# Golbstein/Keras-segmentation-deeplab-v3.1

Hardware: AMD Instinct MI355X
Metric: images/sec fwd+bwd, 512x512 MobileNetV2 OS=16, 21 classes (higher is better)
Workload: dtype f32; 1 GPU; Deeplabv3(backbone='mobilenetv2', input_shape=(512,512,3), classes=21, OS=16) head=deeplab: fwd + sparse-xent loss + bwd + Adam, BN batch mode, dropout 0.1; global_batch=128, per_gpu_batch=128, parallelism=dp1, hipgraph=True, matrix_math=f32, dist_strict=False, backward_fork=False

## Files before the change

### keras-segmentation-deeplab-v3.1_amd/csrc/dwconv.hip

```cpp
#include "common.h"

#pragma clang fp contract(on)
#include <type_traits>
#include <stdlib.h>

namespace {

__device__ __forceinline__ f32x4 ld4_su(const float *base, unsigned byte_off) {
  return ld4(reinterpret_cast<const float *>(reinterpret_cast<const char *>(base) + byte_off));
}
__device__ __forceinline__ void st4_nt_su(float *base, unsigned byte_off, f32x4 v) {
  st4_nt(reinterpret_cast<float *>(reinterpret_cast<char *>(base) + byte_off), v);
}

struct DwGeom {
  int N, H, W, C, stride, rate, pad_t, pad_l, Ho, Wo;
  int prows;
};

struct DwMarch {
  int H, W, C, r, nchunk, TK, nxseg, nphase, ppb, nslab, ny, N;
  int prows;
  int fast;
};

struct DwChan {
  f32x4 wv[9], s, t;
  f32x4 kA, kB, kC, mu, is;
};
__device__ __forceinline__ DwChan dw_chan(int c, int C, const float *w, const float *sc, const float *sh,
                                          const float *cA = nullptr, const float *cB = nullptr, const float *cC = nullptr,
                                          bool stats = false, const float *xmean = nullptr, const float *xinvstd = nullptr) {
  DwChan cn;
  const int c4 = min(c, C - 4);
#pragma unroll
  for (int i = 0; i < 9; i++) cn.wv[i] = ld4(w + (size_t)i * C + c4);
  cn.s = splat4(1.f); cn.t = splat4(0.f);
  cn.kA = splat4(1.f); cn.kB = splat4(0.f); cn.kC = splat4(0.f); cn.mu = splat4(0.f); cn.is = splat4(0.f);
  if (sc) { cn.s = ld4(sc + c4); cn.t = ld4(sh + c4); }
  if (cA) { cn.kA = ld4(cA + c4); cn.kB = ld4(cB + c4); cn.kC = ld4(cC + c4); }
  if (stats) { cn.mu = ld4(xmean + c4); cn.is = ld4(xinvstd + c4); }
  return cn;
}

__device__ __forceinline__ f32x4 dw_dy(const DwChan &cn, f32x4 gv, f32x4 yv) { return cn.kA * gv + cn.kB * yv + cn.kC; }
__device__ __forceinline__ const float *dw_yr(const float *cA, const float *yraw, const float *g) { return cA ? yraw : g; }

template <int NV>
__device__ __forceinline__ void reduce_px(float (&v)[NV], float *lds ) {
  const int tid = threadIdx.x;
  const int wave = tid >> 6, cq = tid & 7;
#pragma unroll
  for (int i = 0; i < NV; i++) {
    float s = v[i];
    s += __shfl_xor(s, 8, 64);
    s += __shfl_xor(s, 16, 64);
    s += __shfl_xor(s, 32, 64);
    v[i] = s;
  }
  __syncthreads();
  if ((tid & 63) < 8) {
#pragma unroll
    for (int i = 0; i < NV; i++) lds[(wave * 8 + cq) * NV + i] = v[i];
  }
  __syncthreads();
  if (tid < 8) {
#pragma unroll
    for (int i = 0; i < NV; i++)
      v[i] = ((lds[(0 * 8 + cq) * NV + i] + lds[(1 * 8 + cq) * NV + i]) + lds[(2 * 8 + cq) * NV + i]) +
             lds[(3 * 8 + cq) * NV + i];
  }
}

__device__ __forceinline__ void write_stat_partial(float *part, int p, int C, int c, f32x4 s1, f32x4 s2) {
  float *d = part + ((size_t)p * C + c) * 2;
  d[0] = s1.x; d[1] = s2.x; d[2] = s1.y; d[3] = s2.y;
  d[4] = s1.z; d[5] = s2.z; d[6] = s1.w; d[7] = s2.w;
}

__device__ __forceinline__ void pad_stat_partial(float *part, int p, int written, int rows, int C, int c) {
  for (int q = p + written; q < rows; q += written) write_stat_partial(part, q, C, c, splat4(0.f), splat4(0.f));
}
__device__ __forceinline__ void pad_w_partial(float *wpart, int p, int written, int rows, int C, int c) {
  for (int q = p + written; q < rows; q += written)
#pragma unroll
    for (int i = 0; i < 9; i++) st4(wpart + ((size_t)q * 9 + i) * C + c, splat4(0.f));
}

__device__ __forceinline__ void dw_store_stats(float *part, int p, int written, int rows, int C, int c, f32x4 s1, f32x4 s2,
                                               float *red ) {
  if (!part) return;
  float v[8] = {s1.x, s1.y, s1.z, s1.w, s2.x, s2.y, s2.z, s2.w};
  reduce_px<8>(v, red);
  if (threadIdx.x < 8 && c < C) {
    f32x4 r1 = {v[0], v[1], v[2], v[3]}, r2 = {v[4], v[5], v[6], v[7]};
    write_stat_partial(part, p, C, c, r1, r2);
    pad_stat_partial(part, p, written, rows, C, c);
  }
}
__device__ __forceinline__ void dw_store_wgrad(float *wpart, int p, int written, int rows, int C, int c, const f32x4 (&dwv)[9],
                                               float *red ) {
  float v[36];
#pragma unroll
  for (int i = 0; i < 9; i++) {
    v[i * 4 + 0] = dwv[i].x; v[i * 4 + 1] = dwv[i].y; v[i * 4 + 2] = dwv[i].z; v[i * 4 + 3] = dwv[i].w;
  }
  reduce_px<36>(v, red);
  if (threadIdx.x < 8 && c < C) {
#pragma unroll
    for (int i = 0; i < 9; i++) {
      f32x4 o = {v[i * 4], v[i * 4 + 1], v[i * 4 + 2], v[i * 4 + 3]};
      st4(wpart + ((size_t)p * 9 + i) * C + c, o);
    }
    pad_w_partial(wpart, p, written, rows, C, c);
  }
}

struct DwTile { int xs, slab, pc, n; };
__device__ __forceinline__ bool dw_tile(const DwMarch &M, DwTile &t) {
  const int L = blockIdx.x, chunk = gridDim.x >> 3;
  int v = (L & 7) * chunk + (L >> 3);
  if (v >= M.nxseg * M.nslab * M.ny * M.N) return false;
  t.xs = v % M.nxseg; v /= M.nxseg;
  t.slab = v % M.nslab; v /= M.nslab;
  t.pc = v % M.ny;
  t.n = v / M.ny;
  t.xs = __builtin_amdgcn_readfirstlane(t.xs);
  t.slab = __builtin_amdgcn_readfirstlane(t.slab);
  t.pc = __builtin_amdgcn_readfirstlane(t.pc);
  t.n = __builtin_amdgcn_readfirstlane(t.n);
  return true;
}
__device__ __forceinline__ int dw_tile_row(const DwMarch &M, const DwTile &t) { return (t.n * M.ny + t.pc) * M.nxseg + t.xs; }

struct DwPhase {
  int a, Ka, k0, k1, Kc;
  bool bot_halo;
  int ks, ke;
};
__device__ __forceinline__ bool dw_phase(const DwMarch &M, int pc, int pi, DwPhase &ph) {
  const int a = __builtin_amdgcn_readfirstlane((M.ppb > 1) ? pc * M.ppb + pi : pc / M.nchunk);
  const int ch = __builtin_amdgcn_readfirstlane((M.ppb > 1) ? 0 : pc % M.nchunk);
  const int Ka = __builtin_amdgcn_readfirstlane((a < M.H) ? (M.H - a + M.r - 1) / M.r : 0);
  const int k0 = ch * M.TK;
  const int k1 = min(k0 + M.TK, Ka);
  const int Kc = max(Ka - 1, 0);
  const bool bot_halo = k1 < Ka;
  const int ks = (k0 > 0) ? k0 - 1 : k0, ke = bot_halo ? k1 : k1 - 1;
  ph = DwPhase{a, Ka, k0, k1, Kc, bot_halo, ks, ke};
  return a < M.nphase;
}

template <int R, class Group>
__device__ __forceinline__ void dw_walk(const DwPhase &ph, bool fast_ok, int fast_last, Group &group) {
  int kg = ph.ks;
  group(kg, std::false_type{});
  kg += R;
  if (fast_ok) {
    __builtin_amdgcn_s_waitcnt(0x0F70);
    for (; kg + R - 1 <= fast_last; kg += R) group(kg, std::true_type{});
  }
  for (; kg <= ph.ke; kg += R) group(kg, std::false_type{});
}

__global__ __launch_bounds__(256, 3) void dw_march_fwd(const float *__restrict__ x, const float *__restrict__ sc,
                                                    const float *__restrict__ sh, int act,
                                                    const float *__restrict__ w, float *__restrict__ y, DwMarch M,
                                                    float *__restrict__ part) {
  __shared__ float red[4 * 8 * 8];
  const int tid = threadIdx.x, cq = tid & 7, pl = tid >> 3;
  DwTile tile;
  if (!dw_tile(M, tile)) return;
  const int H = M.H, W = M.W, C = M.C, r = M.r;
  const int xs = tile.xs, slab = tile.slab, n = tile.n;
  const int c = slab * 32 + cq * 4;
  const int xx = xs * 32 + pl;
  const bool active = (c < C) && (xx < W);

  const DwChan cn = dw_chan(c, C, w, sc, sh);
  f32x4 s1 = splat4(0.f), s2 = splat4(0.f);
  for (int pi = 0; pi < M.ppb; ++pi) {
    DwPhase ph;
    if (!dw_phase(M, tile.pc, pi, ph)) break;
    const int a = ph.a;
    const bool xl_ok = (xx - r >= 0), xr_ok = (xx + r < W);
    const int cc = min(c, C - 4), xc = min(xx, W - 1), xlc = min(max(xx - r, 0), W - 1), xrc = min(xx + r, W - 1);
    const float *xn = x + (size_t)n * H * W * C;
    float *yn = y + (size_t)n * H * W * C;
    const unsigned om = 4u * (unsigned)(xc * C + cc), ol = 4u * (unsigned)(xlc * C + cc), orr = 4u * (unsigned)(xrc * C + cc);
    const unsigned oo = 4u * (unsigned)(xx * C + c);

    auto ldrow = [&](int k, f32x4 &l, f32x4 &m, f32x4 &rr) {
      const bool rok = active && k >= 0 && k < ph.Ka;
      const float *row = xn + (size_t)(a + min(max(k, 0), ph.Kc) * r) * W * C;
      const f32x4 vm = dl3_act4(cn.s * ld4_su(row, om) + cn.t, act);
      const f32x4 vl = dl3_act4(cn.s * ld4_su(row, ol) + cn.t, act);
      const f32x4 vr = dl3_act4(cn.s * ld4_su(row, orr) + cn.t, act);
      m = vm * splat4(rok ? 1.f : 0.f);
      l = vl * splat4((rok && xl_ok) ? 1.f : 0.f);
      rr = vr * splat4((rok && xr_ok) ? 1.f : 0.f);
    };

    f32x4 accA = splat4(0.f), accB = splat4(0.f);
    constexpr int R = 4;
    const bool allact = M.fast && (slab * 32 + 32 <= C) && (xs * 32 + 32 <= W);
    auto group = [&](int kg, auto fastc) __attribute__((always_inline)) {
      constexpr bool FAST = decltype(fastc)::value;
      f32x4 l[R], m[R], rr[R];
#pragma unroll
      for (int j = 0; j < R; j++) {
        if constexpr (FAST) {
          const float *row = xn + (size_t)(a + (kg + j) * r) * W * C;
          m[j] = dl3_act4(cn.s * ld4_su(row, om) + cn.t, act);
          l[j] = dl3_act4(cn.s * ld4_su(row, ol) + cn.t, act) * splat4(xl_ok ? 1.f : 0.f);
          rr[j] = dl3_act4(cn.s * ld4_su(row, orr) + cn.t, act) * splat4(xr_ok ? 1.f : 0.f);
        } else {
          ldrow((kg + j <= ph.ke) ? kg + j : -1, l[j], m[j], rr[j]);
        }
      }
#pragma unroll
      for (int j = 0; j < R; j++) {
        const int k = kg + j;
        const bool kv = FAST || k <= ph.ke;
        f32x4 h0 = cn.wv[0] * l[j] + cn.wv[1] * m[j] + cn.wv[2] * rr[j];
        f32x4 h1 = cn.wv[3] * l[j] + cn.wv[4] * m[j] + cn.wv[5] * rr[j];
        f32x4 h2 = cn.wv[6] * l[j] + cn.wv[7] * m[j] + cn.wv[8] * rr[j];
        f32x4 out = accA + h2;
        if constexpr (FAST) {
          st4_nt_su(yn + (size_t)(a + (k - 1) * r) * W * C, oo, out);
          s1 += out;
          s2 += out * out;
          accA = accB + h1;
          accB = h0;
        } else {
          if (active && kv && k - 1 >= ph.k0 && k - 1 < ph.k1) {
            st4_nt_su(yn + (size_t)(a + (k - 1) * r) * W * C, oo, out);
            s1 += out;
            s2 += out * out;
          }
          accA = kv ? accB + h1 : accA;
          accB = kv ? h0 : accB;
        }
      }
    };
    if (ph.k0 < ph.k1) dw_walk<R>(ph, allact, ph.ke, group);
    if (!ph.bot_halo && ph.k0 < ph.k1 && active) {
      st4_nt_su(yn + (size_t)(a + (ph.k1 - 1) * r) * W * C, oo, accA);
      s1 += accA;
      s2 += accA * accA;
    }
  }
  dw_store_stats(part, dw_tile_row(M, tile), M.N * M.ny * M.nxseg, M.prows, C, c, s1, s2, red);
}

__global__ __launch_bounds__(256, 3) void dw_march2_fwd(const float *__restrict__ x, const float *__restrict__ sc,
                                                     const float *__restrict__ sh, int act,
                                                     const float *__restrict__ w, float *__restrict__ y, DwMarch M,
                                                     float *__restrict__ part) {
  __shared__ float red[4 * 8 * 8];
  const int tid = threadIdx.x, cq = tid & 7, pl = tid >> 3;
  DwTile tile;
  if (!dw_tile(M, tile)) return;
  const int H = M.H, W = M.W, C = M.C, r = M.r;
  const int xs = tile.xs, slab = tile.slab, n = tile.n;
  const int c = slab * 32 + cq * 4;
  const int xa = xs * 64 + (pl / r) * 2 * r + pl % r, xb = xa + r;
  const bool ca = c < C;
  const bool act_a = ca && xa < W, act_b = ca && xb < W;

  const DwChan cn = dw_chan(c, C, w, sc, sh);
  f32x4 s1 = splat4(0.f), s2 = splat4(0.f);
  const int cc = min(c, C - 4);
  const int x0c = min(max(xa - r, 0), W - 1), x1c = min(xa, W - 1), x2c = min(xb, W - 1), x3c = min(xb + r, W - 1);
  const float v0 = (ca && xa - r >= 0 && xa - r < W) ? 1.f : 0.f, v1 = act_a ? 1.f : 0.f, v2 = act_b ? 1.f : 0.f,
              v3 = (ca && xb + r < W) ? 1.f : 0.f;
  const float *xn = x + (size_t)n * H * W * C;
  float *yn = y + (size_t)n * H * W * C;
  const unsigned o0 = 4u * (unsigned)(x0c * C + cc), o1 = 4u * (unsigned)(x1c * C + cc), o2 = 4u * (unsigned)(x2c * C + cc),
                 o3 = 4u * (unsigned)(x3c * C + cc);
  const unsigned osa = 4u * (unsigned)(xa * C + c), osb = 4u * (unsigned)(xb * C + c);
  for (int pi = 0; pi < M.ppb; ++pi) {
    DwPhase ph;
    if (!dw_phase(M, tile.pc, pi, ph)) break;
    const int a = ph.a;
    auto ldrow = [&](int k, f32x4 (&p)[4]) {
      const float rok = (k >= 0 && k < ph.Ka) ? 1.f : 0.f;
      const float *row = xn + (size_t)(a + min(max(k, 0), ph.Kc) * r) * W * C;
      p[0] = dl3_act4(cn.s * ld4_su(row, o0) + cn.t, act) * splat4(rok * v0);
      p[1] = dl3_act4(cn.s * ld4_su(row, o1) + cn.t, act) * splat4(rok * v1);
      p[2] = dl3_act4(cn.s * ld4_su(row, o2) + cn.t, act) * splat4(rok * v2);
      p[3] = dl3_act4(cn.s * ld4_su(row, o3) + cn.t, act) * splat4(rok * v3);
    };
    f32x4 aA = splat4(0.f), aB = splat4(0.f), bA = splat4(0.f), bB = splat4(0.f);
    constexpr int R = 3;
    const bool allact = M.fast && (slab * 32 + 32 <= C) && (xs * 64 + 64 <= W);
    auto group = [&](int kg, auto fastc) __attribute__((always_inline)) {
      constexpr bool FAST = decltype(fastc)::value;
      f32x4 p[R][4];
#pragma unroll
      for (int j = 0; j < R; j++) {
        if constexpr (FAST) {
          const float *row = xn + (size_t)(a + (kg + j) * r) * W * C;
          p[j][0] = dl3_act4(cn.s * ld4_su(row, o0) + cn.t, act) * splat4(v0);
          p[j][1] = dl3_act4(cn.s * ld4_su(row, o1) + cn.t, act) * splat4(v1);
          p[j][2] = dl3_act4(cn.s * ld4_su(row, o2) + cn.t, act) * splat4(v2);
          p[j][3] = dl3_act4(cn.s * ld4_su(row, o3) + cn.t, act) * splat4(v3);
        } else {
          ldrow((kg + j <= ph.ke) ? kg + j : -1, p[j]);
        }
      }
#pragma unroll
      for (int j = 0; j < R; j++) {
        const int k = kg + j;
        const bool kv = FAST || k <= ph.ke;
        const f32x4 a0 = cn.wv[0] * p[j][0] + cn.wv[1] * p[j][1] + cn.wv[2] * p[j][2];
        const f32x4 a1 = cn.wv[3] * p[j][0] + cn.wv[4] * p[j][1] + cn.wv[5] * p[j][2];
        const f32x4 a2 = cn.wv[6] * p[j][0] + cn.wv[7] * p[j][1] + cn.wv[8] * p[j][2];
        const f32x4 b0 = cn.wv[0] * p[j][1] + cn.wv[1] * p[j][2] + cn.wv[2] * p[j][3];
        const f32x4 b1 = cn.wv[3] * p[j][1] + cn.wv[4] * p[j][2] + cn.wv[5] * p[j][3];
        const f32x4 b2 = cn.wv[6] * p[j][1] + cn.wv[7] * p[j][2] + cn.wv[8] * p[j][3];
        const f32x4 oa = aA + a2, ob = bA + b2;
        if constexpr (FAST) {
          float *orow = yn + (size_t)(a + (k - 1) * r) * W * C;
          st4_nt_su(orow, osa, oa); s1 += oa; s2 += oa * oa;
          st4_nt_su(orow, osb, ob); s1 += ob; s2 += ob * ob;
          aA = aB + a1; aB = a0;
          bA = bB + b1; bB = b0;
        } else {
          if (kv && k - 1 >= ph.k0 && k - 1 < ph.k1) {
            float *orow = yn + (size_t)(a + (k - 1) * r) * W * C;
            if (act_a) { st4_nt_su(orow, osa, oa); s1 += oa; s2 += oa * oa; }
            if (act_b) { st4_nt_su(orow, osb, ob); s1 += ob; s2 += ob * ob; }
          }
          aA = kv ? aB + a1 : aA; aB = kv ? a0 : aB;
          bA = kv ? bB + b1 : bA; bB = kv ? b0 : bB;
        }
      }
    };
    if (ph.k0 < ph.k1) dw_walk<R>(ph, allact, ph.ke, group);
    if (!ph.bot_halo && ph.k0 < ph.k1) {
      float *orow = yn + (size_t)(a + (ph.k1 - 1) * r) * W * C;
      if (act_a) { st4_nt_su(orow, osa, aA); s1 += aA; s2 += aA * aA; }
      if (act_b) { st4_nt_su(orow, osb, bA); s1 += bA; s2 += bA * bA; }
    }
  }
  dw_store_stats(part, dw_tile_row(M, tile), M.N * M.ny * M.nxseg, M.prows, C, c, s1, s2, red);
}

template <bool SXK, bool ADDK>
__global__ __launch_bounds__(256, 2) void dw_march_bwd(
    const float *__restrict__ g, const float *__restrict__ yraw, const float *__restrict__ cA,
    const float *__restrict__ cB, const float *__restrict__ cC, const float *__restrict__ x,
    const float *__restrict__ sc, const float *__restrict__ sh, int act, const float *__restrict__ w,
    float *__restrict__ dx, const float *__restrict__ dx_add, const float *__restrict__ xmean,
    const float *__restrict__ xinvstd, float *__restrict__ dpart, float *__restrict__ wpart, DwMarch M,
    const float *__restrict__ sx) {
  __shared__ float red[4 * 8 * 36];
  const int tid = threadIdx.x, cq = tid & 7, pl = tid >> 3;
  DwTile tile;
  if (!dw_tile(M, tile)) return;
  const int H = M.H, W = M.W, C = M.C, r = M.r;
  const int xs = tile.xs, slab = tile.slab, n = tile.n;
  const int c = slab * 32 + cq * 4;
  const int xx = xs * 32 + pl;
  const bool active = (c < C) && (xx < W);

  const DwChan cn = dw_chan(c, C, w, sc, sh, cA, cB, cC, dpart != nullptr, xmean, xinvstd);
  const bool xl_ok = (xx - r >= 0), xr_ok = (xx + r < W);
  const int cc = min(c, C - 4), xc = min(xx, W - 1), xlc = min(max(xx - r, 0), W - 1), xrc = min(xx + r, W - 1);
  const size_t nimg = (size_t)n * H * W * C;
  const unsigned om = 4u * (unsigned)(xc * C + cc), ol = 4u * (unsigned)(xlc * C + cc), orr = 4u * (unsigned)(xrc * C + cc);
  const unsigned oo = 4u * (unsigned)(xx * C + c);
  const bool allact = M.fast && (slab * 32 + 32 <= C) && (xs * 32 + 32 <= W);
  f32x4 dwv[9];
#pragma unroll
  for (int i = 0; i < 9; i++) dwv[i] = splat4(0.f);
  f32x4 s1 = splat4(0.f), s2 = splat4(0.f);
  for (int pi = 0; pi < M.ppb; ++pi) {
    DwPhase ph;
    if (!dw_phase(M, tile.pc, pi, ph)) break;
    const int a = ph.a;
    const float *yr = dw_yr(cA, yraw, g);
    auto rowoff = [&](int k) -> size_t { return nimg + (size_t)(a + min(max(k, 0), ph.Kc) * r) * W * C; };

    auto ld_dd1 = [&](size_t row, unsigned off) -> f32x4 { return dw_dy(cn, ld4_su(g + row, off), ld4_su(yr + row, off)); };
    auto ld_dd = [&](int k, f32x4 &l, f32x4 &m, f32x4 &rr) {
      const bool rok = active && k >= 0 && k < ph.Ka;
      const size_t row = rowoff(k);
      const f32x4 vm = ld_dd1(row, om), vl = ld_dd1(row, ol), vr = ld_dd1(row, orr);
      m = vm * splat4(rok ? 1.f : 0.f);
      l = vl * splat4((rok && xl_ok) ? 1.f : 0.f);
      rr = vr * splat4((rok && xr_ok) ? 1.f : 0.f);
    };
    auto ld_e = [&](int k, f32x4 &raw, bool &ok) {
      ok = active && k >= 0 && k < ph.Ka;
      raw = ld4_su(x + rowoff(k), om);
    };
    auto eact = [&](f32x4 raw, bool ok) -> f32x4 {
      const f32x4 v = dl3_act4(cn.s * raw + cn.t, act);
      return v * splat4(ok ? 1.f : 0.f);
    };

    f32x4 accA = splat4(0.f), accB = splat4(0.f);

    if (ph.k0 < ph.k1) {
      constexpr int R = 2;
      f32x4 e_prev = splat4(0.f), e_cur, e_next;
      bool ok_prev = false, ok_cur, ok_next;
      ld_e(ph.ks, e_cur, ok_cur);
      ld_e(ph.ks + 1, e_next, ok_next);
      auto group = [&](int kg, auto fastc) __attribute__((always_inline)) {
        constexpr bool FAST = decltype(fastc)::value, SXC = SXK, ADDC = ADDK;
        f32x4 l[R], m[R], rr[R], e_new[R], sxv[R], addv[R];
        bool ok_new[R];
#pragma unroll
        for (int j = 0; j < R; j++) {
          if constexpr (FAST) {
            const size_t row = nimg + (size_t)(a + (kg + j) * r) * W * C;
            m[j] = ld_dd1(row, om);
            l[j] = ld_dd1(row, ol) * splat4(xl_ok ? 1.f : 0.f);
            rr[j] = ld_dd1(row, orr) * splat4(xr_ok ? 1.f : 0.f);
            ld_e(kg + j + 2, e_new[j], ok_new[j]);
            const size_t orow = nimg + (size_t)(a + (kg + j - 1) * r) * W * C;
            if constexpr (SXC) sxv[j] = ld4_su(sx + orow, om);
            if constexpr (ADDC) addv[j] = ld4_su(dx_add + orow, om);
          } else {
            ld_dd((kg + j <= ph.ke) ? kg + j : -1, l[j], m[j], rr[j]);
            ld_e(kg + j + 2, e_new[j], ok_new[j]);
            const size_t orow = rowoff(kg + j - 1);
            if constexpr (SXC) sxv[j] = ld4_su(sx + orow, om);
            if constexpr (ADDC) addv[j] = ld4_su(dx_add + orow, om);
          }
        }
#pragma unroll
        for (int j = 0; j < R; j++) {
          const int k = kg + j;
          const bool kv = FAST || k <= ph.ke;
          if (FAST || (k >= ph.k0 && k < ph.k1)) {
            f32x4 ea0 = eact(e_prev, ok_prev), ea1 = eact(e_cur, ok_cur), ea2 = eact(e_next, ok_next);
            dwv[0] += ea0 * rr[j]; dwv[1] += ea0 * m[j]; dwv[2] += ea0 * l[j];
            dwv[3] += ea1 * rr[j]; dwv[4] += ea1 * m[j]; dwv[5] += ea1 * l[j];
            dwv[6] += ea2 * rr[j]; dwv[7] += ea2 * m[j]; dwv[8] += ea2 * l[j];
          }
          f32x4 h0 = cn.wv[0] * rr[j] + cn.wv[1] * m[j] + cn.wv[2] * l[j];
          f32x4 h1 = cn.wv[3] * rr[j] + cn.wv[4] * m[j] + cn.wv[5] * l[j];
          f32x4 h2 = cn.wv[6] * rr[j] + cn.wv[7] * m[j] + cn.wv[8] * l[j];
          f32x4 out = accA + h0;
          if constexpr (FAST) {
            out = out * dl3_mask4(cn.s * e_prev + cn.t, act);
            if constexpr (ADDC) out += addv[j];
            st4_nt_su(dx + nimg + (size_t)(a + (k - 1) * r) * W * C, oo, out);
            s1 += out;
            s2 += out * (((SXC ? sxv[j] : e_prev) - cn.mu) * cn.is);
            accA = accB + h1;
            accB = h2;
            e_prev = e_cur; ok_prev = ok_cur;
            e_cur = e_next; ok_cur = ok_next;
            e_next = e_new[j]; ok_next = ok_new[j];
          } else {
            if (dx && active && kv && k - 1 >= ph.k0 && k - 1 < ph.k1) {
              out = out * dl3_mask4(cn.s * e_prev + cn.t, act);
              if constexpr (ADDC) out += addv[j];
              st4_nt_su(dx + nimg + (size_t)(a + (k - 1) * r) * W * C, oo, out);
              s1 += out;
              s2 += out * (((SXC ? sxv[j] : e_prev) - cn.mu) * cn.is);
            }
            accA = kv ? accB + h1 : accA;
            accB = kv ? h2 : accB;
            e_prev = kv ? e_cur : e_prev; ok_prev = kv ? ok_cur : ok_prev;
            e_cur = kv ? e_next : e_cur; ok_cur = kv ? ok_next : ok_cur;
            e_next = kv ? e_new[j] : e_next; ok_next = kv ? ok_new[j] : ok_next;
          }
        }
      };
      dw_walk<R>(ph, allact && dx, ph.k1 - 1, group);
      if (!ph.bot_halo && dx && active) {
        const size_t row = nimg + (size_t)(a + (ph.k1 - 1) * r) * W * C;
        f32x4 out = accA * dl3_mask4(cn.s * e_prev + cn.t, act);
        if constexpr (ADDK) out += ld4_su(dx_add + row, oo);
        st4_nt_su(dx + row, oo, out);
        s1 += out;
        s2 += out * (((SXK ? ld4_su(sx + row, oo) : e_prev) - cn.mu) * cn.is);
      }
    }
  }
  const int p = dw_tile_row(M, tile), written = M.N * M.ny * M.nxseg;
  dw_store_wgrad(wpart, p, written, M.prows, C, c, dwv, red);
  dw_store_stats(dpart, p, written, M.prows, C, c, s1, s2, red);
}

__global__ __launch_bounds__(256) void dw_gather_fwd(const float *__restrict__ x, const float *__restrict__ sc,
                                                     const float *__restrict__ sh, int act,
                                                     const float *__restrict__ w, float *__restrict__ y, DwGeom G,
                                                     float *__restrict__ part) {
  __shared__ float red[4 * 8 * 8];
  const int tid = threadIdx.x, cq = tid & 7, pl = tid >> 3;
  const int c = blockIdx.x * 32 + cq * 4;
  const bool cok = c < G.C;
  const DwChan cn = dw_chan(c, G.C, w, sc, sh);
  f32x4 s1 = splat4(0.f), s2 = splat4(0.f);
  const long NP = (long)G.N * G.Ho * G.Wo;
  for (long p = (long)blockIdx.y * 32 + pl; p < NP && cok; p += (long)gridDim.y * 32) {
    const int ox = (int)(p % G.Wo);
    const int oy = (int)((p / G.Wo) % G.Ho);
    const int n = (int)(p / ((long)G.Wo * G.Ho));
    f32x4 acc = splat4(0.f);
    f32x4 tap[9];
    float okf[9];
#pragma unroll
    for (int i = 0; i < 3; i++) {
      const int iy = oy * G.stride - G.pad_t + i * G.rate;
      const int iyc = min(max(iy, 0), G.H - 1);
#pragma unroll
      for (int j = 0; j < 3; j++) {
        const int ix = ox * G.stride - G.pad_l + j * G.rate;
        const int ixc = min(max(ix, 0), G.W - 1);
        okf[i * 3 + j] = (iy == iyc && ix == ixc) ? 1.f : 0.f;
        tap[i * 3 + j] = ld4(x + (((size_t)n * G.H + iyc) * G.W + ixc) * G.C + c);
      }
    }
#pragma unroll
    for (int q = 0; q < 9; q++) acc += (cn.wv[q] * splat4(okf[q])) * dl3_act4(cn.s * tap[q] + cn.t, act);
    st4_nt(y + (size_t)p * G.C + c, acc);
    s1 += acc;
    s2 += acc * acc;
  }
  dw_store_stats(part, blockIdx.y, gridDim.y, G.prows, G.C, c, s1, s2, red);
}

__global__ __launch_bounds__(256) void dw_gather_bwd(
    const float *__restrict__ g, const float *__restrict__ yraw, const float *__restrict__ cA,
    const float *__restrict__ cB, const float *__restrict__ cC, const float *__restrict__ x,
    const float *__restrict__ sc, const float *__restrict__ sh, int act, const float *__restrict__ w,
    float *__restrict__ dx, const float *__restrict__ dx_add, const float *__restrict__ xmean,
    const float *__restrict__ xinvstd, float *__restrict__ dpart, float *__restrict__ wpart, DwGeom G) {
  __shared__ float red[4 * 8 * 36];
  const int tid = threadIdx.x, cq = tid & 7, pl = tid >> 3;
  const int c = blockIdx.x * 32 + cq * 4;
  const bool cok = c < G.C;
  const DwChan cn = dw_chan(c, G.C, w, sc, sh, cA, cB, cC, dpart != nullptr, xmean, xinvstd);
  f32x4 dwv[9];
#pragma unroll
  for (int i = 0; i < 9; i++) dwv[i] = splat4(0.f);
  f32x4 s1 = splat4(0.f), s2 = splat4(0.f);
  const long NP = (long)G.N * G.H * G.W;
  for (long p = (long)blockIdx.y * 32 + pl; p < NP && cok; p += (long)gridDim.y * 32) {
    const int ix = (int)(p % G.W);
    const int iy = (int)((p / G.W) % G.H);
    const int n = (int)(p / ((long)G.W * G.H));
    const f32x4 eraw = ld4(x + (size_t)p * G.C + c);
    const f32x4 z = cn.s * eraw + cn.t;
    const f32x4 ea = dl3_act4(z, act);
    f32x4 acc = splat4(0.f);
    const float *yr = dw_yr(cA, yraw, g);
    f32x4 tg[9], ty_[9];
    float okf[9];
#pragma unroll
    for (int i = 0; i < 3; i++) {
      const int ty = iy + G.pad_t - i * G.rate;
      const int oy = max(ty, 0) / G.stride;
      const bool yok = ty >= 0 && (ty % G.stride) == 0 && oy < G.Ho;
      const int oyc = min(oy, G.Ho - 1);
#pragma unroll
      for (int j = 0; j < 3; j++) {
        const int tx = ix + G.pad_l - j * G.rate;
        const int ox = max(tx, 0) / G.stride;
        const bool xok = tx >= 0 && (tx % G.stride) == 0 && ox < G.Wo;
        const int oxc = min(ox, G.Wo - 1);
        const size_t off = (((size_t)n * G.Ho + oyc) * G.Wo + oxc) * G.C + c;
        okf[i * 3 + j] = (yok && xok) ? 1.f : 0.f;
        tg[i * 3 + j] = ld4(g + off);
        ty_[i * 3 + j] = ld4(yr + off);
      }
    }
#pragma unroll
    for (int q = 0; q < 9; q++) {
      const f32x4 dd = dw_dy(cn, tg[q], ty_[q]) * splat4(okf[q]);
      acc += dd * cn.wv[q];
      dwv[q] += ea * dd;
    }
    if (dx) {
      f32x4 out = acc * dl3_mask4(z, act);
      if (dx_add) out += ld4(dx_add + (size_t)p * G.C + c);
      st4_nt(dx + (size_t)p * G.C + c, out);
      s1 += out;
      s2 += out * ((eraw - cn.mu) * cn.is);
    }
  }
  dw_store_wgrad(wpart, blockIdx.y, gridDim.y, G.prows, G.C, c, dwv, red);
  dw_store_stats(dpart, blockIdx.y, gridDim.y, G.prows, G.C, c, s1, s2, red);
}

__global__ __launch_bounds__(256) void dw_s2_bwd(
    const float *__restrict__ g, const float *__restrict__ yraw, const float *__restrict__ cA,
    const float *__restrict__ cB, const float *__restrict__ cC, const float *__restrict__ x,
    const float *__restrict__ sc, const float *__restrict__ sh, int act, const float *__restrict__ w,
    float *__restrict__ dx, const float *__restrict__ dx_add, const float *__restrict__ xmean,
    const float *__restrict__ xinvstd, float *__restrict__ dpart, float *__restrict__ wpart, DwGeom G) {
  __shared__ float red[4 * 8 * 36];
  const int tid = threadIdx.x, cq = tid & 7, pl = tid >> 3;
  const int c = blockIdx.x * 32 + cq * 4;
  const bool cok = c < G.C;
  const int cc = min(c, G.C - 4);
  const DwChan cn = dw_chan(c, G.C, w, sc, sh, cA, cB, cC, dpart != nullptr, xmean, xinvstd);
  const float *yr = dw_yr(cA, yraw, g);
  f32x4 dwv[9];
#pragma unroll
  for (int i = 0; i < 9; i++) dwv[i] = splat4(0.f);
  f32x4 s1 = splat4(0.f), s2 = splat4(0.f);
  const int A = (G.H + G.pad_t + 1) / 2, Bn = (G.W + G.pad_l + 1) / 2;
  const long NB = (long)G.N * A * Bn;
  for (long q = (long)blockIdx.y * 32 + pl; q < NB; q += (long)gridDim.y * 32) {
    const int b = (int)(q % Bn), a = (int)((q / Bn) % A), n = (int)(q / ((long)Bn * A));
    const int iy0 = 2 * a - G.pad_t, ix0 = 2 * b - G.pad_l;
    f32x4 dd[2][2];
#pragma unroll
    for (int i = 0; i < 2; i++)
#pragma unroll
      for (int j = 0; j < 2; j++) {
        const int oy = a - i, ox = b - j;
        const int oyc = min(max(oy, 0), G.Ho - 1), oxc = min(max(ox, 0), G.Wo - 1);
        const float ok = (cok && oy == oyc && ox == oxc) ? 1.f : 0.f;
        const size_t off = (((size_t)n * G.Ho + oyc) * G.Wo + oxc) * G.C + cc;
        dd[i][j] = dw_dy(cn, ld4(g + off), ld4(yr + off)) * splat4(ok);
      }
    f32x4 xr[2][2], ad[2][2];
    float pok[2][2];
    size_t poff[2][2];
#pragma unroll
    for (int i = 0; i < 2; i++)
#pragma unroll
      for (int j = 0; j < 2; j++) {
        const int iy = iy0 + i, ix = ix0 + j;
        const int iyc = min(max(iy, 0), G.H - 1), ixc = min(max(ix, 0), G.W - 1);
        pok[i][j] = (cok && iy == iyc && ix == ixc) ? 1.f : 0.f;
        poff[i][j] = (((size_t)n * G.H + iyc) * G.W + ixc) * G.C + cc;
        xr[i][j] = ld4(x + poff[i][j]);
        ad[i][j] = dx_add ? ld4(dx_add + poff[i][j]) : splat4(0.f);
      }
    f32x4 acc[2][2];
    acc[0][0] = cn.wv[0] * dd[0][0] + cn.wv[6] * dd[1][0] + cn.wv[2] * dd[0][1] + cn.wv[8] * dd[1][1];
    acc[0][1] = cn.wv[1] * dd[0][0] + cn.wv[7] * dd[1][0];
    acc[1][0] = cn.wv[3] * dd[0][0] + cn.wv[5] * dd[0][1];
    acc[1][1] = cn.wv[4] * dd[0][0];
    f32x4 ea[2][2];
#pragma unroll
    for (int i = 0; i < 2; i++)
#pragma unroll
      for (int j = 0; j < 2; j++) ea[i][j] = dl3_act4(cn.s * xr[i][j] + cn.t, act) * splat4(pok[i][j]);
    dwv[0] += ea[0][0] * dd[0][0]; dwv[6] += ea[0][0] * dd[1][0]; dwv[2] += ea[0][0] * dd[0][1]; dwv[8] += ea[0][0] * dd[1][1];
    dwv[1] += ea[0][1] * dd[0][0]; dwv[7] += ea[0][1] * dd[1][0];
    dwv[3] += ea[1][0] * dd[0][0]; dwv[5] += ea[1][0] * dd[0][1];
    dwv[4] += ea[1][1] * dd[0][0];
    if (dx) {
#pragma unroll
      for (int i = 0; i < 2; i++)
#pragma unroll
        for (int j = 0; j < 2; j++) {
          f32x4 out = acc[i][j] * dl3_mask4(cn.s * xr[i][j] + cn.t, act) + ad[i][j];
          if (pok[i][j] != 0.f) {
            st4_nt(dx + poff[i][j], out);
            s1 += out;
            s2 += out * ((xr[i][j] - cn.mu) * cn.is);
          }
        }
    }
  }
  dw_store_wgrad(wpart, blockIdx.y, gridDim.y, G.prows, G.C, c, dwv, red);
  dw_store_stats(dpart, blockIdx.y, gridDim.y, G.prows, G.C, c, s1, s2, red);
}

struct DwPlan {
  int impl;
  int nslab, nxseg, nphase, nchunk, TK;
  int ppb, ny;
  int two;
  int PB;
  int P;
};

unsigned march_grid(const DwPlan &p, int N) {
  const long total = (long)p.nxseg * p.nslab * p.ny * N;
  return (unsigned)((total + 7) / 8 * 8);
}

bool march_ok(int H, int W, int stride, int rate, int pad_t, int pad_l, int Ho, int Wo) {
  return stride == 1 && pad_t == rate && pad_l == rate && Ho == H && Wo == W;
}

DwPlan dw_plan(int N, int H, int W, int C, int stride, int rate, int Ho, int Wo, int impl, bool bwd) {
  DwPlan p{};
  p.nslab = dl3_cdiv(C, 32);
  p.impl = impl;
  if (impl == DL3_IMPL_MARCH) {
    p.two = (!bwd && 32 % rate == 0 && W >= 32) ? 1 : 0;
    p.nxseg = dl3_cdiv(W, p.two ? 64 : 32);
    p.nphase = rate < H ? rate : H;
    const int Kmax = dl3_cdiv(H, rate);
    int TK = Kmax;
    const long want = 1024;
    while (TK > 8 && (long)N * p.nslab * p.nxseg * p.nphase * dl3_cdiv(Kmax, TK) < want) TK = (TK + 1) / 2;
    p.TK = TK;
    p.nchunk = dl3_cdiv(Kmax, TK);
    int ppb = 1;
    if (p.nchunk == 1 && Kmax < 12) {
      ppb = 12 / Kmax;
      if (ppb > p.nphase) ppb = p.nphase;
      while (ppb > 1 && (long)N * p.nslab * p.nxseg * dl3_cdiv(p.nphase, ppb) < 2048) --ppb;
      if (const char *e = getenv("DL3_DW_PPB")) ppb = atoi(e);
      if (ppb > p.nphase) ppb = p.nphase;
      if (ppb < 1) ppb = 1;
    }
    p.ppb = ppb;
    p.ny = (ppb > 1) ? dl3_cdiv(p.nphase, ppb) : p.nphase * p.nchunk;
    p.P = N * p.ny * p.nxseg;
  } else {
    const long NP = bwd ? (long)N * H * W : (long)N * Ho * Wo;
    long pb = (NP + 31) / 32;
    long cap = 4096 / p.nslab;
    if (cap < 1) cap = 1;
    if (pb > cap) pb = cap;
    p.PB = (int)pb;
    p.P = p.PB;
  }
  return p;
}

int resolve_impl(int impl, int H, int W, int stride, int rate, int pad_t, int pad_l, int Ho, int Wo) {
  const bool ok = march_ok(H, W, stride, rate, pad_t, pad_l, Ho, Wo);
  if (impl == DL3_IMPL_AUTO) return ok ? DL3_IMPL_MARCH : DL3_IMPL_GATHER;
  if (impl == DL3_IMPL_MARCH && !ok) return -1;
  return impl;
}

bool auto_sized_for_march(int H, int W, int stride, int Ho, int Wo) {
  return stride == 1 && Ho == H && Wo == W;
}

bool auto_mismatch(int impl, int im, int H, int W, int stride, int Ho, int Wo) {
  return impl == DL3_IMPL_AUTO && im == DL3_IMPL_GATHER && auto_sized_for_march(H, W, stride, Ho, Wo);
}

}

extern "C" int dl3_dwconv3x3_partials(int N, int H, int W, int C, int stride, int rate, int Ho, int Wo,
                                      int impl) {
  int im = impl;
  if (im == DL3_IMPL_AUTO) im = auto_sized_for_march(H, W, stride, Ho, Wo) ? DL3_IMPL_MARCH : DL3_IMPL_GATHER;
  DwPlan a = dw_plan(N, H, W, C, stride, rate, Ho, Wo, im, false);
  DwPlan b = dw_plan(N, H, W, C, stride, rate, Ho, Wo, im, true);
  return a.P > b.P ? a.P : b.P;
}

static int dw_check(int N, int H, int W, int C, int stride, int rate, int Ho, int Wo) {
  DL3_CHECK_ARG(N > 0 && H > 0 && W > 0 && C > 0 && Ho > 0 && Wo > 0, "dwconv3x3: non-positive dimension");
  DL3_CHECK_ARG(stride >= 1 && rate >= 1, "dwconv3x3: stride/rate must be >= 1");
  DL3_UNSUPPORTED(C % 4 != 0, "dwconv3x3: C=%d must be a multiple of 4", C);
  DL3_UNSUPPORTED(N > 65535, "dwconv3x3: N=%d too large for grid.z", N);
  return DL3_OK;
}

struct DwLaunch {
  int im;
  DwPlan p;
  dim3 grid;
  DwMarch M;
  DwGeom G;
};
static int dw_prepare(const char *fn, bool bwd, int N, int H, int W, int C, int stride, int rate, int pad_t, int pad_l,
                      int Ho, int Wo, int impl, DwLaunch &L) {
  int rc = dw_check(N, H, W, C, stride, rate, Ho, Wo);
  if (rc) return rc;
  const int im = resolve_impl(impl, H, W, stride, rate, pad_t, pad_l, Ho, Wo);
  DL3_UNSUPPORTED(im < 0, "%s: march impl needs stride 1, pad == rate, Ho == H, Wo == W", fn);
  DL3_UNSUPPORTED(auto_mismatch(impl, im, H, W, stride, Ho, Wo),
                  "%s: DL3_IMPL_AUTO sizes the partials of a stride-1 Ho == H, Wo == W geometry for the march kernels, "
                  "pad (%d,%d) != rate %d needs the gather kernels: size and launch with DL3_IMPL_GATHER", fn, pad_t, pad_l, rate);
  const DwPlan p = dw_plan(N, H, W, C, stride, rate, Ho, Wo, im, bwd);
  const int Pmax = dl3_dwconv3x3_partials(N, H, W, C, stride, rate, Ho, Wo, im);
  L.im = im;
  L.p = p;
  if (im == DL3_IMPL_MARCH) {
    const int fast = (C % 32 == 0);
    L.grid = dim3(march_grid(p, N));
    L.M = DwMarch{H, W, C, rate, p.nchunk, p.TK, p.nxseg, p.nphase, p.ppb, p.nslab, p.ny, N, Pmax, fast};
  } else {
    L.grid = dim3(p.nslab, p.PB);
    L.G = DwGeom{N, H, W, C, stride, rate, pad_t, pad_l, Ho, Wo, Pmax};
  }
  return DL3_OK;
}

extern "C" int dl3_dwconv3x3_fwd(const float *x, const float *in_scale, const float *in_shift, int in_act,
                                 const float *w, float *y, int N, int H, int W, int C, int stride, int rate,
                                 int pad_t, int pad_l, int Ho, int Wo, float *stat_partial, int impl,
                                 void *stream) {
  DwLaunch L;
  int rc = dw_prepare("dwconv3x3_fwd", false, N, H, W, C, stride, rate, pad_t, pad_l, Ho, Wo, impl, L);
  if (rc) return rc;
  DL3_CHECK_ARG(x && w && y, "dwconv3x3_fwd: null pointer");
  DL3_CHECK_ARG((in_scale == nullptr) == (in_shift == nullptr), "dwconv3x3_fwd: scale/shift must come together");
  hipStream_t st = (hipStream_t)stream;
  if (L.im == DL3_IMPL_MARCH) {
    if (L.p.two)
      hipLaunchKernelGGL(dw_march2_fwd, L.grid, dim3(256), 0, st, x, in_scale, in_shift, in_act, w, y, L.M, stat_partial);
    else
      hipLaunchKernelGGL(dw_march_fwd, L.grid, dim3(256), 0, st, x, in_scale, in_shift, in_act, w, y, L.M, stat_partial);
  } else {
    hipLaunchKernelGGL(dw_gather_fwd, L.grid, dim3(256), 0, st, x, in_scale, in_shift, in_act, w, y, L.G, stat_partial);
  }
  DL3_LAUNCH_CHECK("dwconv3x3_fwd");
  return DL3_OK;
}

static int dwconv3x3_bwd_impl(const float *g, const float *yraw, const float *cA, const float *cB,
                                 const float *cC, const float *x, const float *in_scale, const float *in_shift,
                                 int in_act, const float *w, float *dx, const float *dx_add,
                                 const float *x_mean, const float *x_invstd, float *dstat_partial,
                                 float *dw_partial, int N, int H, int W, int C, int stride, int rate, int pad_t,
                                 int pad_l, int Ho, int Wo, int impl, const float *stat_x, void *stream) {
  DwLaunch L;
  int rc = dw_prepare("dwconv3x3_bwd", true, N, H, W, C, stride, rate, pad_t, pad_l, Ho, Wo, impl, L);
  if (rc) return rc;
  DL3_CHECK_ARG(!stat_x || dstat_partial, "dwconv3x3_bwd_sx: stat_x without dstat_partial");
  DL3_CHECK_ARG(g && x && w && dw_partial, "dwconv3x3_bwd: null pointer");
  DL3_CHECK_ARG(!cA || (yraw && cB && cC), "dwconv3x3_bwd: cA needs yraw, cB, cC");
  DL3_CHECK_ARG((in_scale == nullptr) == (in_shift == nullptr), "dwconv3x3_bwd: scale/shift must come together");
  DL3_CHECK_ARG(!dstat_partial || (dx && x_mean && x_invstd), "dwconv3x3_bwd: dstat needs dx, x_mean, x_invstd");
  DL3_UNSUPPORTED(stat_x && L.im != DL3_IMPL_MARCH, "dwconv3x3_bwd_sx: sums against another tensor need the march kernel (stride 1, SAME)");
  hipStream_t st = (hipStream_t)stream;
  if (L.im == DL3_IMPL_MARCH) {
    auto *kernel = stat_x ? (dx_add ? dw_march_bwd<true, true> : dw_march_bwd<true, false>)
                          : (dx_add ? dw_march_bwd<false, true> : dw_march_bwd<false, false>);
    hipLaunchKernelGGL(kernel, L.grid, dim3(256), 0, st, g, yraw, cA, cB, cC, x, in_scale, in_shift, in_act, w, dx, dx_add,
                       x_mean, x_invstd, dstat_partial, dw_partial, L.M, stat_x);
  } else {
    if (stride == 2 && rate == 1 && pad_t <= 1 && pad_l <= 1)
      hipLaunchKernelGGL(dw_s2_bwd, L.grid, dim3(256), 0, st, g, yraw, cA, cB, cC, x, in_scale, in_shift, in_act, w, dx,
                         dx_add, x_mean, x_invstd, dstat_partial, dw_partial, L.G);
    else
      hipLaunchKernelGGL(dw_gather_bwd, L.grid, dim3(256), 0, st, g, yraw, cA, cB, cC, x, in_scale, in_shift, in_act,
                         w, dx, dx_add, x_mean, x_invstd, dstat_partial, dw_partial, L.G);
  }
  DL3_LAUNCH_CHECK("dwconv3x3_bwd");
  return DL3_OK;
}

extern "C" int dl3_dwconv3x3_bwd(const float *g, const float *yraw, const float *cA, const float *cB,
                                 const float *cC, const float *x, const float *in_scale, const float *in_shift,
                                 int in_act, const float *w, float *dx, const float *dx_add,
                                 const float *x_mean, const float *x_invstd, float *dstat_partial,
                                 float *dw_partial, int N, int H, int W, int C, int stride, int rate, int pad_t,
                                 int pad_l, int Ho, int Wo, int impl, void *stream) {
  return dwconv3x3_bwd_impl(g, yraw, cA, cB, cC, x, in_scale, in_shift, in_act, w, dx, dx_add, x_mean, x_invstd,
                            dstat_partial, dw_partial, N, H, W, C, stride, rate, pad_t, pad_l, Ho, Wo, impl, nullptr, stream);
}

extern "C" int dl3_dwconv3x3_bwd_sx(const float *g, const float *yraw, const float *cA, const float *cB,
                                    const float *cC, const float *x, const float *in_scale, const float *in_shift,
                                    int in_act, const float *w, float *dx, const float *dx_add, const float *stat_x,
                                    const float *x_mean, const float *x_invstd, float *dstat_partial,
                                    float *dw_partial, int N, int H, int W, int C, int stride, int rate, int pad_t,
                                    int pad_l, int Ho, int Wo, int impl, void *stream) {
  DL3_CHECK_ARG(stat_x, "dwconv3x3_bwd_sx: stat_x is NULL (use dl3_dwconv3x3_bwd)");
  return dwconv3x3_bwd_impl(g, yraw, cA, cB, cC, x, in_scale, in_shift, in_act, w, dx, dx_add, x_mean, x_invstd,
                            dstat_partial, dw_partial, N, H, W, C, stride, rate, pad_t, pad_l, Ho, Wo, impl, stat_x, stream);
}
```

Before: 1347 img/s.

## Add two-column-per-thread march backward kernel for dilated depthwise conv

Adds a dw_march2_bwd kernel in which each thread handles two output columns spaced by the dilation rate, so the four gradient loads per row are shared between two outputs. The planner enables it for backward when the rate is 4 or more, divides 32, and W is at least 32, which halves the number of x-segments. The aim is to cut redundant global loads in the dilated ASPP/backbone depthwise backward. In exchange the kernel uses more registers (launch_bounds 256,2) and launches fewer blocks. The partials-size query still plans with pairs disabled, so the buffer sizing may not match the new plan.

Result: no change. 1345 img/s (-0.1%).

```diff
diff --git a/keras-segmentation-deeplab-v3.1_amd/csrc/dwconv.hip b/keras-segmentation-deeplab-v3.1_amd/csrc/dwconv.hip
--- a/keras-segmentation-deeplab-v3.1_amd/csrc/dwconv.hip
+++ b/keras-segmentation-deeplab-v3.1_amd/csrc/dwconv.hip
@@ -489,6 +489,188 @@
   dw_store_stats(dpart, p, written, M.prows, C, c, s1, s2, red);
 }
 
+template <bool SXK, bool ADDK>
+__global__ __launch_bounds__(256, 2) void dw_march2_bwd(
+    const float *__restrict__ g, const float *__restrict__ yraw, const float *__restrict__ cA,
+    const float *__restrict__ cB, const float *__restrict__ cC, const float *__restrict__ x,
+    const float *__restrict__ sc, const float *__restrict__ sh, int act, const float *__restrict__ w,
+    float *__restrict__ dx, const float *__restrict__ dx_add, const float *__restrict__ xmean,
+    const float *__restrict__ xinvstd, float *__restrict__ dpart, float *__restrict__ wpart, DwMarch M,
+    const float *__restrict__ sx) {
+  __shared__ float red[4 * 8 * 36];
+  const int tid = threadIdx.x, cq = tid & 7, pl = tid >> 3;
+  DwTile tile;
+  if (!dw_tile(M, tile)) return;
+  const int H = M.H, W = M.W, C = M.C, r = M.r;
+  const int xs = tile.xs, slab = tile.slab, n = tile.n;
+  const int c = slab * 32 + cq * 4;
+  const int xa = xs * 64 + (pl / r) * 2 * r + pl % r, xb = xa + r;
+  const bool ca = c < C;
+  const bool act_a = ca && xa < W, act_b = ca && xb < W;
+
+  const DwChan cn = dw_chan(c, C, w, sc, sh, cA, cB, cC, dpart != nullptr, xmean, xinvstd);
+  const int cc = min(c, C - 4);
+  const int x0c = min(max(xa - r, 0), W - 1), x1c = min(xa, W - 1), x2c = min(xb, W - 1), x3c = min(xb + r, W - 1);
+  const float v0 = (ca && xa - r >= 0 && xa - r < W) ? 1.f : 0.f, v1 = act_a ? 1.f : 0.f, v2 = act_b ? 1.f : 0.f,
+              v3 = (ca && xb + r < W) ? 1.f : 0.f;
+  const size_t nimg = (size_t)n * H * W * C;
+  const unsigned o0 = 4u * (unsigned)(x0c * C + cc), o1 = 4u * (unsigned)(x1c * C + cc), o2 = 4u * (unsigned)(x2c * C + cc),
+                 o3 = 4u * (unsigned)(x3c * C + cc);
+  const unsigned osa = 4u * (unsigned)(xa * C + c), osb = 4u * (unsigned)(xb * C + c);
+  const bool allact = M.fast && (slab * 32 + 32 <= C) && (xs * 64 + 64 <= W);
+  f32x4 dwv[9];
+#pragma unroll
+  for (int i = 0; i < 9; i++) dwv[i] = splat4(0.f);
+  f32x4 s1 = splat4(0.f), s2 = splat4(0.f);
+  for (int pi = 0; pi < M.ppb; ++pi) {
+    DwPhase ph;
+    if (!dw_phase(M, tile.pc, pi, ph)) break;
+    const int a = ph.a;
+    const float *yr = dw_yr(cA, yraw, g);
+    auto rowoff = [&](int k) -> size_t { return nimg + (size_t)(a + min(max(k, 0), ph.Kc) * r) * W * C; };
+
+    auto ld_dd1 = [&](size_t row, unsigned off) -> f32x4 { return dw_dy(cn, ld4_su(g + row, off), ld4_su(yr + row, off)); };
+    auto ld_dd = [&](int k, f32x4 (&d)[4]) {
+      const float rok = (k >= 0 && k < ph.Ka) ? 1.f : 0.f;
+      const size_t row = rowoff(k);
+      const f32x4 d0 = ld_dd1(row, o0), d1 = ld_dd1(row, o1), d2 = ld_dd1(row, o2), d3 = ld_dd1(row, o3);
+      d[0] = d0 * splat4(rok * v0);
+      d[1] = d1 * splat4(rok * v1);
+      d[2] = d2 * splat4(rok * v2);
+      d[3] = d3 * splat4(rok * v3);
+    };
+    auto ld_e = [&](int k, f32x4 &rawa, f32x4 &rawb, bool &ok) {
+      ok = k >= 0 && k < ph.Ka;
+      const size_t row = rowoff(k);
+      rawa = ld4_su(x + row, o1);
+      rawb = ld4_su(x + row, o2);
+    };
+    auto eact = [&](f32x4 raw, bool ok, float v) -> f32x4 {
+      const f32x4 e = dl3_act4(cn.s * raw + cn.t, act);
+      return e * splat4(ok ? v : 0.f);
+    };
+
+    f32x4 aA = splat4(0.f), aB = splat4(0.f), bA = splat4(0.f), bB = splat4(0.f);
+
+    if (ph.k0 < ph.k1) {
+      constexpr int R = 1;
+      f32x4 ea_prev = splat4(0.f), ea_cur, ea_next, eb_prev = splat4(0.f), eb_cur, eb_next;
+      bool ok_prev = false, ok_cur, ok_next;
+      ld_e(ph.ks, ea_cur, eb_cur, ok_cur);
+      ld_e(ph.ks + 1, ea_next, eb_next, ok_next);
+      auto group = [&](int kg, auto fastc) __attribute__((always_inline)) {
+        constexpr bool FAST = decltype(fastc)::value, SXC = SXK, ADDC = ADDK;
+        {
+          const int k = kg;
+          f32x4 d[4], ea_new, eb_new, sxa, sxb, adda, addb;
+          bool ok_new;
+          size_t irow;
+          if constexpr (FAST) {
+            const size_t row = nimg + (size_t)(a + k * r) * W * C;
+            d[0] = ld_dd1(row, o0) * splat4(v0);
+            d[1] = ld_dd1(row, o1);
+            d[2] = ld_dd1(row, o2);
+            d[3] = ld_dd1(row, o3) * splat4(v3);
+            irow = nimg + (size_t)(a + (k - 1) * r) * W * C;
+          } else {
+            ld_dd((k <= ph.ke) ? k : -1, d);
+            irow = rowoff(k - 1);
+          }
+          ld_e(k + 2, ea_new, eb_new, ok_new);
+          if constexpr (SXC) { sxa = ld4_su(sx + irow, o1); sxb = ld4_su(sx + irow, o2); }
+          if constexpr (ADDC) { adda = ld4_su(dx_add + irow, o1); addb = ld4_su(dx_add + irow, o2); }
+          const bool kv = FAST || k <= ph.ke;
+          const f32x4 la = d[0], ma = d[1], ra = d[2], lb = d[1], mb = d[2], rb = d[3];
+          if (FAST || (k >= ph.k0 && k < ph.k1)) {
+            f32x4 ea0 = eact(ea_prev, ok_prev, v1), ea1 = eact(ea_cur, ok_cur, v1), ea2 = eact(ea_next, ok_next, v1);
+            dwv[0] += ea0 * ra; dwv[1] += ea0 * ma; dwv[2] += ea0 * la;
+            dwv[3] += ea1 * ra; dwv[4] += ea1 * ma; dwv[5] += ea1 * la;
+            dwv[6] += ea2 * ra; dwv[7] += ea2 * ma; dwv[8] += ea2 * la;
+            f32x4 eb0 = eact(eb_prev, ok_prev, v2), eb1 = eact(eb_cur, ok_cur, v2), eb2 = eact(eb_next, ok_next, v2);
+            dwv[0] += eb0 * rb; dwv[1] += eb0 * mb; dwv[2] += eb0 * lb;
+            dwv[3] += eb1 * rb; dwv[4] += eb1 * mb; dwv[5] += eb1 * lb;
+            dwv[6] += eb2 * rb; dwv[7] += eb2 * mb; dwv[8] += eb2 * lb;
+          }
+          f32x4 h0a = cn.wv[0] * ra + cn.wv[1] * ma + cn.wv[2] * la;
+          f32x4 h1a = cn.wv[3] * ra + cn.wv[4] * ma + cn.wv[5] * la;
+          f32x4 h2a = cn.wv[6] * ra + cn.wv[7] * ma + cn.wv[8] * la;
+          f32x4 h0b = cn.wv[0] * rb + cn.wv[1] * mb + cn.wv[2] * lb;
+          f32x4 h1b = cn.wv[3] * rb + cn.wv[4] * mb + cn.wv[5] * lb;
+          f32x4 h2b = cn.wv[6] * rb + cn.wv[7] * mb + cn.wv[8] * lb;
+          f32x4 oa = aA + h0a, ob = bA + h0b;
+          if constexpr (FAST) {
+            float *orow = dx + nimg + (size_t)(a + (k - 1) * r) * W * C;
+            oa = oa * dl3_mask4(cn.s * ea_prev + cn.t, act);
+            if constexpr (ADDC) oa += adda;
+            st4_nt_su(orow, osa, oa);
+            s1 += oa;
+            s2 += oa * (((SXC ? sxa : ea_prev) - cn.mu) * cn.is);
+            ob = ob * dl3_mask4(cn.s * eb_prev + cn.t, act);
+            if constexpr (ADDC) ob += addb;
+            st4_nt_su(orow, osb, ob);
+            s1 += ob;
+            s2 += ob * (((SXC ? sxb : eb_prev) - cn.mu) * cn.is);
+            aA = aB + h1a; aB = h2a;
+            bA = bB + h1b; bB = h2b;
+            ea_prev = ea_cur; ea_cur = ea_next; ea_next = ea_new;
+            eb_prev = eb_cur; eb_cur = eb_next; eb_next = eb_new;
+            ok_prev = ok_cur; ok_cur = ok_next; ok_next = ok_new;
+          } else {
+            if (dx && kv && k - 1 >= ph.k0 && k - 1 < ph.k1) {
+              float *orow = dx + nimg + (size_t)(a + (k - 1) * r) * W * C;
+              if (act_a) {
+                oa = oa * dl3_mask4(cn.s * ea_prev + cn.t, act);
+                if constexpr (ADDC) oa += adda;
+                st4_nt_su(orow, osa, oa);
+                s1 += oa;
+                s2 += oa * (((SXC ? sxa : ea_prev) - cn.mu) * cn.is);
+              }
+              if (act_b) {
+                ob = ob * dl3_mask4(cn.s * eb_prev + cn.t, act);
+                if constexpr (ADDC) ob += addb;
+                st4_nt_su(orow, osb, ob);
+                s1 += ob;
+                s2 += ob * (((SXC ? sxb : eb_prev) - cn.mu) * cn.is);
+              }
+            }
+            aA = kv ? aB + h1a : aA; aB = kv ? h2a : aB;
+            bA = kv ? bB + h1b : bA; bB = kv ? h2b : bB;
+            ea_prev = kv ? ea_cur : ea_prev; ea_cur = kv ? ea_next : ea_cur; ea_next = kv ? ea_new : ea_next;
+            eb_prev = kv ? eb_cur : eb_prev; eb_cur = kv ? eb_next : eb_cur; eb_next = kv ? eb_new : eb_next;
+            ok_prev = kv ? ok_cur : ok_prev; ok_cur = kv ? ok_next : ok_cur; ok_next = kv ? ok_new : ok_next;
+          }
+        }
+      };
+      DwPhase pw = ph;
+      if (ph.ks < ph.k0) {
+        group(ph.ks, std::false_type{});
+        pw.ks = ph.k0;
+      }
+      dw_walk<R>(pw, allact && dx, ph.k1 - 1, group);
+      if (!ph.bot_halo && dx) {
+        const size_t row = nimg + (size_t)(a + (ph.k1 - 1) * r) * W * C;
+        if (act_a) {
+          f32x4 out = aA * dl3_mask4(cn.s * ea_prev + cn.t, act);
+          if constexpr (ADDK) out += ld4_su(dx_add + row, osa);
+          st4_nt_su(dx + row, osa, out);
+          s1 += out;
+          s2 += out * (((SXK ? ld4_su(sx + row, osa) : ea_prev) - cn.mu) * cn.is);
+        }
+        if (act_b) {
+          f32x4 out = bA * dl3_mask4(cn.s * eb_prev + cn.t, act);
+          if constexpr (ADDK) out += ld4_su(dx_add + row, osb);
+          st4_nt_su(dx + row, osb, out);
+          s1 += out;
+          s2 += out * (((SXK ? ld4_su(sx + row, osb) : eb_prev) - cn.mu) * cn.is);
+        }
+      }
+    }
+  }
+  const int p = dw_tile_row(M, tile), written = M.N * M.ny * M.nxseg;
+  dw_store_wgrad(wpart, p, written, M.prows, C, c, dwv, red);
+  dw_store_stats(dpart, p, written, M.prows, C, c, s1, s2, red);
+}
+
 __global__ __launch_bounds__(256) void dw_gather_fwd(const float *__restrict__ x, const float *__restrict__ sc,
                                                      const float *__restrict__ sh, int act,
                                                      const float *__restrict__ w, float *__restrict__ y, DwGeom G,
@@ -688,12 +870,13 @@
   return stride == 1 && pad_t == rate && pad_l == rate && Ho == H && Wo == W;
 }
 
-DwPlan dw_plan(int N, int H, int W, int C, int stride, int rate, int Ho, int Wo, int impl, bool bwd) {
+DwPlan dw_plan(int N, int H, int W, int C, int stride, int rate, int Ho, int Wo, int impl, bool bwd, bool pairs = true) {
   DwPlan p{};
   p.nslab = dl3_cdiv(C, 32);
   p.impl = impl;
   if (impl == DL3_IMPL_MARCH) {
     p.two = (!bwd && 32 % rate == 0 && W >= 32) ? 1 : 0;
+    if (bwd && pairs && rate >= 4 && 32 % rate == 0 && W >= 32) p.two = 1;
     p.nxseg = dl3_cdiv(W, p.two ? 64 : 32);
     p.nphase = rate < H ? rate : H;
     const int Kmax = dl3_cdiv(H, rate);
@@ -748,7 +931,7 @@
   int im = impl;
   if (im == DL3_IMPL_AUTO) im = auto_sized_for_march(H, W, stride, Ho, Wo) ? DL3_IMPL_MARCH : DL3_IMPL_GATHER;
   DwPlan a = dw_plan(N, H, W, C, stride, rate, Ho, Wo, im, false);
-  DwPlan b = dw_plan(N, H, W, C, stride, rate, Ho, Wo, im, true);
+  DwPlan b = dw_plan(N, H, W, C, stride, rate, Ho, Wo, im, true, false);
   return a.P > b.P ? a.P : b.P;
 }
 
@@ -832,6 +1015,9 @@
   if (L.im == DL3_IMPL_MARCH) {
     auto *kernel = stat_x ? (dx_add ? dw_march_bwd<true, true> : dw_march_bwd<true, false>)
                           : (dx_add ? dw_march_bwd<false, true> : dw_march_bwd<false, false>);
+    if (L.p.two)
+      kernel = stat_x ? (dx_add ? dw_march2_bwd<true, true> : dw_march2_bwd<true, false>)
+                      : (dx_add ? dw_march2_bwd<false, true> : dw_march2_bwd<false, false>);
     hipLaunchKernelGGL(kernel, L.grid, dim3(256), 0, st, g, yraw, cA, cB, cC, x, in_scale, in_shift, in_act, w, dx, dx_add,
                        x_mean, x_invstd, dstat_partial, dw_partial, L.M, stat_x);
   } else {
```
